# mkshing/e4t-diffusion

Hardware: NVIDIA H100
Metric: E4T pretrain images/sec @512^2 bs16 SD-v1.4 (higher is better)
Workload: dtype bf16

## Files before the change

e4t-diffusion_b200/csrc/attention_wgmma.cu:

```cuda
#include "attention.cuh"
#include "wgmma.cuh"

static constexpr int kWgThreads = 384;
static constexpr int kFwdStages = 3;
static constexpr int kTile128 = 128 * 128;
static constexpr int kTile64 = 64 * 128;
static constexpr size_t kMaxSmem = 227 * 1024;

__device__ __forceinline__ constexpr uint64_t kstep(int k, uint32_t panel) {
  return (uint64_t)((k / 4) * (panel >> 4) + 2 * (k % 4));
}

__device__ __forceinline__ uint8_t* align1024(uint8_t* p) {
  return p + ((1024u - (smem_u32(p) & 1023u)) & 1023u);
}

template <int DH>
struct FwdSmem {
  static constexpr int P = (DH + 63) / 64;
  static constexpr uint32_t kTile = P * kTile128;
  static constexpr uint32_t kStage = 2 * kTile;
  static constexpr uint32_t kOffBar = kTile + kFwdStages * kStage;
  static constexpr size_t bytes = 1024 + kOffBar + 8 * (1 + 2 * kFwdStages);
  static constexpr uint32_t kLboV = P > 1 ? kTile128 : kTile64;
  static_assert(bytes <= kMaxSmem, "forward shared memory");
};

template <int DH>
struct BwdSmem {
  static constexpr int P = (DH + 63) / 64, BQ = 64;
  static constexpr int kStages = P > 1 ? 2 : 3;
  static constexpr uint32_t kKV = P * kTile128;
  static constexpr uint32_t kQ = P * kTile64;
  static constexpr uint32_t kStage = 2 * kQ;
  static constexpr uint32_t kOffQ = 2 * kKV;
  static constexpr uint32_t kOffdS = kOffQ + kStages * kStage;
  static constexpr uint32_t kOffdQ = kOffdS + 2 * kTile128;
  static constexpr uint32_t kdQBytes = BQ * DH * 4;
  static constexpr uint32_t kOffL = kOffdQ + 2 * kdQBytes;
  static constexpr uint32_t kOffBar = kOffL + kStages * 2 * BQ * 4;
  static constexpr size_t bytes = 1024 + kOffBar + 8 * (1 + 2 * kStages + 4);
  static constexpr uint32_t kLboK = P > 1 ? kTile128 : kTile64;
  static_assert(kOffdQ % 128 == 0 && kdQBytes % 128 == 0 && kOffL % 16 == 0 && kOffBar % 8 == 0, "smem layout");
  static_assert(bytes <= kMaxSmem, "backward shared memory");
};

__device__ __forceinline__ void fwd_softmax(float (&s)[64], float (&m)[2], float (&l)[2], float (&alpha)[2], float sl2) {
#pragma unroll
  for (int hr = 0; hr < 2; ++hr) {
    float mx = -INFINITY;
#pragma unroll
    for (int j = 0; j < 16; ++j) mx = fmaxf(mx, fmaxf(s[4 * j + 2 * hr], s[4 * j + 2 * hr + 1]));
    mx = fmaxf(mx, __shfl_xor_sync(0xffffffffu, mx, 1));
    mx = fmaxf(mx, __shfl_xor_sync(0xffffffffu, mx, 2));
    const float mnew = fmaxf(m[hr], mx * sl2);
    alpha[hr] = ex2_approx(m[hr] - mnew);
    m[hr] = mnew;
    float rs = 0.f;
#pragma unroll
    for (int j = 0; j < 16; ++j)
#pragma unroll
      for (int e = 0; e < 2; ++e) {
        const float p = ex2_approx(fmaf(s[4 * j + 2 * hr + e], sl2, -mnew));
        s[4 * j + 2 * hr + e] = p;
        rs += p;
      }
    l[hr] = l[hr] * alpha[hr] + rs;
  }
}

template <int NJ>
__device__ __forceinline__ void pack_acc(const float* s, uint32_t* p) {
#pragma unroll
  for (int i = 0; i < 2 * NJ; ++i) p[i] = pack_bf16(s[2 * i], s[2 * i + 1]);
}

template <int DH>
__global__ void __launch_bounds__(kWgThreads, 1)
attn_wgmma_fwd_kernel(const __grid_constant__ CUtensorMap mapQ, const __grid_constant__ CUtensorMap mapK,
                      const __grid_constant__ CUtensorMap mapV, const AttnArgs a) {
  using L = FwdSmem<DH>;
  constexpr int KS = (DH + 15) / 16, NO = DH;
  constexpr uint32_t kStage = L::kStage;
  extern __shared__ __align__(1024) uint8_t smem_raw[];
  uint8_t* smem = align1024(smem_raw);
  uint64_t* q_bar = reinterpret_cast<uint64_t*>(smem + L::kOffBar);
  uint64_t* full_bar = q_bar + 1;
  uint64_t* empty_bar = full_bar + kFwdStages;
  const int wg = threadIdx.x >> 7;
  const int b = blockIdx.z, h = blockIdx.y, q0 = blockIdx.x * 128;
  const int nblk = a.M / 128;
  if (threadIdx.x == 0) {
    tma_prefetch_desc(&mapQ);
    tma_prefetch_desc(&mapK);
    tma_prefetch_desc(&mapV);
    mbar_init(q_bar, 1);
    for (int i = 0; i < kFwdStages; ++i) {
      mbar_init(&full_bar[i], 1);
      mbar_init(&empty_bar[i], 256);
    }
    fence_mbar_init();
  }
  __syncthreads();

  if (wg == 0) {
    setmaxnreg_dec<24>();
    if (threadIdx.x != 0) return;
    mbar_expect_tx(q_bar, L::kTile);
#pragma unroll
    for (int pn = 0; pn < L::P; ++pn) tma_load_4d(smem + pn * kTile128, &mapQ, q_bar, 64 * pn, h, q0, b);
    int s = 0;
    uint32_t ph = 0;
    for (int j = 0; j < nblk; ++j) {
      mbar_wait(&empty_bar[s], ph ^ 1u);
// ... 141 lines not shown
    }
    for (int i = 0; i < 2; ++i) {
      mbar_init(&ds_full[i], 256);
      mbar_init(&ds_empty[i], 128);
    }
    fence_mbar_init();
  }
  __syncthreads();
  const uint32_t s0 = smem_u32(smem);

  if (wg == 0) {
    setmaxnreg_dec<72>();
    auto load_block = [&](int i) {
      const int s = i % kBwdStages;
      mbar_wait(&empty_bar[s], ((uint32_t)(i / kBwdStages) & 1u) ^ 1u);
      uint8_t* sQ = smem + kOffQ + s * kStage;
      mbar_expect_tx(&full_bar[s], kStage + 2 * BQ * 4);
#pragma unroll
      for (int pn = 0; pn < L::P; ++pn) {
        tma_load_4d(sQ + pn * kTile64, &mapQ, &full_bar[s], 64 * pn, h, i * BQ, b);
        tma_load_4d(sQ + L::kQ + pn * kTile64, &mapdO, &full_bar[s], 64 * pn, h, i * BQ, b);
      }
      bulk_load_1d(sL + s * 2 * BQ, a.LSE + bh * a.N + i * BQ, BQ * 4, &full_bar[s]);
      bulk_load_1d(sL + s * 2 * BQ + BQ, a.Dv + bh * a.N + i * BQ, BQ * 4, &full_bar[s]);
    };
    if (threadIdx.x == 0) {
      mbar_expect_tx(kv_bar, 2 * L::kKV);
#pragma unroll
      for (int pn = 0; pn < L::P; ++pn) {
        tma_load_4d(smem + pn * kTile128, &mapK, kv_bar, 64 * pn, h, k0, b);
        tma_load_4d(smem + L::kKV + pn * kTile128, &mapV, kv_bar, 64 * pn, h, k0, b);
      }
      for (int i = 0; i < kBwdStages - 1 && i < nq; ++i) load_block(i);
    }
    __syncwarp();
    const uint64_t descS = wgmma_desc(s0 + kOffdS, kTile64, 1024);
    const uint64_t descK = wgmma_desc(s0, L::kLboK, 1024);
    mbar_wait(kv_bar, 0);
    float dq[NO / 2];
    for (int i = 0; i < nq; ++i) {
      const int buf = i & 1;
      if (threadIdx.x == 0 && i + kBwdStages - 1 < nq) load_block(i + kBwdStages - 1);
      __syncwarp();
      mbar_wait(&ds_full[buf], (uint32_t)(i >> 1) & 1u);
      const uint64_t da = descS + (uint64_t)(buf * (kTile128 >> 4));
      wgmma_fence();
#pragma unroll
      for (int kk = 0; kk < 8; ++kk)
        Wgmma<NO, 1, 1>::mma(dq, da + (uint64_t)(kk * (2048 >> 4)), descK + (uint64_t)(kk * (2048 >> 4)), kk > 0);
      wgmma_commit();
      wgmma_wait<0>();
      reg_fence<NO / 2>(dq);
      mbar_arrive(&ds_empty[buf]);
      if (threadIdx.x == 0) tma_store_wait_read<1>();
      named_bar_sync(1, 128);
      float* stg = reinterpret_cast<float*>(smem + kOffdQ + buf * kdQBytes);
#pragma unroll
      for (int hr = 0; hr < 2; ++hr) {
        float* row = stg + (16 * warp + (lane >> 2) + 8 * hr) * DH + 2 * (lane & 3);
#pragma unroll
        for (int dt = 0; dt < DH / 8; ++dt)
          *reinterpret_cast<float2*>(row + 8 * dt) =
              make_float2(dq[4 * dt + 2 * hr] * a.scale, dq[4 * dt + 2 * hr + 1] * a.scale);
      }
      fence_proxy_async_smem();
      named_bar_sync(1, 128);
      if (threadIdx.x == 0) {
        tma_reduce_add_3d(&mapdQ, stg, h * DH, i * BQ, b);
        tma_store_commit();
      }
    }
    if (threadIdx.x == 0) tma_store_wait_all();
    return;
  }

  setmaxnreg_inc<216>();
  const int cw = wg - 1;
  const uint64_t descKa = wgmma_desc(s0 + kTile64 * cw, 16, 1024);
  const uint64_t descVa = wgmma_desc(s0 + L::kKV + kTile64 * cw, 16, 1024);
  const uint64_t descQk = wgmma_desc(s0 + kOffQ, 16, 1024);
  const uint64_t descQm = wgmma_desc(s0 + kOffQ, kTile64, 1024);
  const float sl2 = a.scale * kLog2e;
  float st[32], dpt[32], dk[NO / 2], dv[NO / 2];
  uint32_t pp[16], ps[16];
#pragma unroll
  for (int i = 0; i < NO / 2; ++i) dk[i] = dv[i] = 0.f;
  const int r0 = 64 * cw + 16 * warp + (lane >> 2);
  mbar_wait(kv_bar, 0);
  for (int i = 0; i < nq; ++i) {
    const int s = i % kBwdStages, buf = i & 1;
    mbar_wait(&full_bar[s], (uint32_t)(i / kBwdStages) & 1u);
    const uint64_t so = (uint64_t)(s * (kStage >> 4));
    reg_fence<32>(st);
    reg_fence<32>(dpt);
    wgmma_fence();
#pragma unroll
    for (int k = 0; k < KS; ++k)
      Wgmma<64, 0, 0>::mma(st, descKa + kstep(k, kTile128), descQk + so + kstep(k, kTile64), k > 0);
    wgmma_commit();
#pragma unroll
    for (int k = 0; k < KS; ++k)
      Wgmma<64, 0, 0>::mma(dpt, descVa + kstep(k, kTile128), descQk + so + (L::kQ >> 4) + kstep(k, kTile64), k > 0);
    wgmma_commit();
    const float* l_s = sL + s * 2 * BQ + 2 * (lane & 3);
    wgmma_wait<1>();
    reg_fence<32>(st);
#pragma unroll
    for (int j = 0; j < 8; ++j) {
      const float2 l = *reinterpret_cast<const float2*>(l_s + 8 * j);
      const float l0 = l.x * kLog2e, l1 = l.y * kLog2e;
      st[4 * j] = ex2_approx(fmaf(st[4 * j], sl2, -l0));
      st[4 * j + 1] = ex2_approx(fmaf(st[4 * j + 1], sl2, -l1));
      st[4 * j + 2] = ex2_approx(fmaf(st[4 * j + 2], sl2, -l0));
      st[4 * j + 3] = ex2_approx(fmaf(st[4 * j + 3], sl2, -l1));
    }
    pack_acc<8>(st, pp);
    wgmma_wait<0>();
    reg_fence<32>(dpt);
#pragma unroll
    for (int j = 0; j < 8; ++j) {
      const float2 d = *reinterpret_cast<const float2*>(l_s + BQ + 8 * j);
      dpt[4 * j] = st[4 * j] * (dpt[4 * j] - d.x);
      dpt[4 * j + 1] = st[4 * j + 1] * (dpt[4 * j + 1] - d.y);
      dpt[4 * j + 2] = st[4 * j + 2] * (dpt[4 * j + 2] - d.x);
      dpt[4 * j + 3] = st[4 * j + 3] * (dpt[4 * j + 3] - d.y);
    }
    pack_acc<8>(dpt, ps);
    mbar_wait(&ds_empty[buf], ((uint32_t)(i >> 1) & 1u) ^ 1u);
    uint8_t* sdS = smem + kOffdS + buf * kTile128;
#pragma unroll
    for (int j = 0; j < 8; ++j) {
      *reinterpret_cast<uint32_t*>(sdS + sw128_off(r0, j) + 4 * (lane & 3)) = ps[2 * j];
      *reinterpret_cast<uint32_t*>(sdS + sw128_off(r0 + 8, j) + 4 * (lane & 3)) = ps[2 * j + 1];
    }
    fence_proxy_async_smem();
    mbar_arrive(&ds_full[buf]);
    reg_fence<NO / 2>(dk);
    reg_fence<NO / 2>(dv);
    wgmma_fence();
#pragma unroll
    for (int kq = 0; kq < 4; ++kq)
      WgmmaRS<NO, 1>::mma(dv, pp + 4 * kq, descQm + so + (uint64_t)((L::kQ >> 4) + kq * (2048 >> 4)), 1);
#pragma unroll
    for (int kq = 0; kq < 4; ++kq) WgmmaRS<NO, 1>::mma(dk, ps + 4 * kq, descQm + so + (uint64_t)(kq * (2048 >> 4)), 1);
    wgmma_commit();
    wgmma_wait<0>();
    reg_fence<NO / 2>(dk);
    reg_fence<NO / 2>(dv);
    reg_fence_u32<16>(pp);
    reg_fence_u32<16>(ps);
    mbar_arrive(&empty_bar[s]);
  }
#pragma unroll
  for (int hr = 0; hr < 2; ++hr) {
    const int key = k0 + r0 + 8 * hr;
    bf16* dkr = a.dK + b * a.dk_bs + (long long)key * a.lddk + h * DH + 2 * (lane & 3);
    bf16* dvr = a.dV + b * a.dv_bs + (long long)key * a.lddv + h * DH + 2 * (lane & 3);
#pragma unroll
    for (int dt = 0; dt < DH / 8; ++dt) {
      *reinterpret_cast<uint32_t*>(dkr + 8 * dt) = pack_bf16(dk[4 * dt + 2 * hr] * a.scale, dk[4 * dt + 2 * hr + 1] * a.scale);
      *reinterpret_cast<uint32_t*>(dvr + 8 * dt) = pack_bf16(dv[4 * dt + 2 * hr], dv[4 * dt + 2 * hr + 1]);
    }
  }
}

bool attn_wgmma_shape_ok(int B, int H, int N, int M, int dh) {
  if (!(dh == 40 || dh == 64 || dh == 80) || N < 512 || M < 512 || N % 128 != 0 || M % 128 != 0) return false;
  if (dh == 40) return true;
  int sms = 0, dev = 0;
  cudaGetDevice(&dev);
  cudaDeviceGetAttribute(&sms, cudaDevAttrMultiProcessorCount, dev);
  if (sms <= 0) sms = 132;
  return 2LL * (N / 128) * H * B >= sms;
}

static int head_map(CUtensorMap* m, const bf16* p, const AttnArgs& a, int tokens, long long ld, long long bs, int rows) {
  E4T_CHECK(((uintptr_t)p & 15) == 0 && ld % 8 == 0 && bs % 8 == 0,
            "attention (wgmma): tensors must be 16-byte aligned with strides that are multiples of 8 elements");
  const uint64_t dims[4] = {(uint64_t)a.dh, (uint64_t)a.H, (uint64_t)tokens, (uint64_t)a.B};
  const uint64_t str[3] = {(uint64_t)a.dh * 2, (uint64_t)ld * 2, (uint64_t)bs * 2};
  const uint32_t box[4] = {64, 1, (uint32_t)rows, 1};
  return e4t_tmap_encode(m, p, 4, dims, str, box, 2);
}

int attn_wgmma_fwd(const AttnArgs& a, cudaStream_t st) {
  CUtensorMap mQ, mK, mV;
  if (int e = head_map(&mQ, a.Q, a, a.N, a.ldq, a.q_bs, 128)) return e;
  if (int e = head_map(&mK, a.K, a, a.M, a.ldk, a.k_bs, 128)) return e;
  if (int e = head_map(&mV, a.V, a, a.M, a.ldv, a.v_bs, 128)) return e;
  E4T_CHECK(a.ldo % 2 == 0 && a.o_bs % 2 == 0, "attention (wgmma): output strides must be even");
  const size_t smem = a.dh == 40 ? FwdSmem<40>::bytes : a.dh == 64 ? FwdSmem<64>::bytes : FwdSmem<80>::bytes;
  auto kernel = a.dh == 40   ? attn_wgmma_fwd_kernel<40>
                : a.dh == 64 ? attn_wgmma_fwd_kernel<64>
                             : attn_wgmma_fwd_kernel<80>;
  E4T_CUDA(cudaFuncSetAttribute(kernel, cudaFuncAttributeMaxDynamicSharedMemorySize, (int)smem));
  kernel<<<dim3(a.N / 128, a.H, a.B), kWgThreads, smem, st>>>(mQ, mK, mV, a);
  E4T_COUNT_LAUNCH();
  E4T_LAUNCH_CHECK();
  return 0;
}

int attn_wgmma_bwd(const AttnArgs& a, cudaStream_t st) {
  CUtensorMap mQ, mK, mV, mdO, mdQ;
  if (int e = head_map(&mQ, a.Q, a, a.N, a.ldq, a.q_bs, 64)) return e;
  if (int e = head_map(&mK, a.K, a, a.M, a.ldk, a.k_bs, 128)) return e;
  if (int e = head_map(&mV, a.V, a, a.M, a.ldv, a.v_bs, 128)) return e;
  if (int e = head_map(&mdO, a.dO, a, a.N, a.lddo, a.do_bs, 64)) return e;
  {
    const uint64_t C = (uint64_t)a.H * a.dh;
    const uint64_t dims[3] = {C, (uint64_t)a.N, (uint64_t)a.B};
    const uint64_t str[2] = {C * 4, (uint64_t)a.N * C * 4};
    const uint32_t box[3] = {(uint32_t)a.dh, 64, 1};
    E4T_CHECK(((uintptr_t)a.dQacc & 15) == 0 && ((uintptr_t)a.LSE & 15) == 0 && ((uintptr_t)a.Dv & 15) == 0,
              "attention (wgmma): LSE, D and dQ scratch must be 16-byte aligned");
    if (int e = e4t_tmap_encode(&mdQ, a.dQacc, 3, dims, str, box, 4, 0)) return e;
  }
  E4T_CHECK(a.lddk % 2 == 0 && a.dk_bs % 2 == 0 && a.lddv % 2 == 0 && a.dv_bs % 2 == 0,
            "attention (wgmma): gradient strides must be even");
  const size_t smem = a.dh == 40 ? BwdSmem<40>::bytes : a.dh == 64 ? BwdSmem<64>::bytes : BwdSmem<80>::bytes;
  auto kernel = a.dh == 40   ? attn_wgmma_bwd_kernel<40>
                : a.dh == 64 ? attn_wgmma_bwd_kernel<64>
                             : attn_wgmma_bwd_kernel<80>;
  E4T_CUDA(cudaFuncSetAttribute(kernel, cudaFuncAttributeMaxDynamicSharedMemorySize, (int)smem));
  kernel<<<dim3(a.M / 128, a.H, a.B), kWgThreads, smem, st>>>(mQ, mK, mV, mdO, mdQ, a);
  E4T_COUNT_LAUNCH();
  E4T_LAUNCH_CHECK();
  return 0;
}
```

e4t-diffusion_b200/csrc/common.cuh:

```cuda
#pragma once
#include <cuda.h>
#include <cuda_runtime.h>
#include <cuda_bf16.h>
#include <stdint.h>
#include <stdio.h>
#include <string.h>

typedef __nv_bfloat16 bf16;

extern thread_local char g_e4t_err[512];
int e4t_set_error(const char* fmt, ...);

#define E4T_CHECK(cond, ...)                                   \
  do {                                                         \
    if (!(cond)) return e4t_set_error(__VA_ARGS__);            \
  } while (0)

#define E4T_CUDA(call)                                                                  \
  do {                                                                                  \
    cudaError_t _e = (call);                                                            \
    if (_e != cudaSuccess)                                                              \
      return e4t_set_error("%s:%d CUDA error %s: %s", __FILE__, __LINE__, #call,        \
                           cudaGetErrorString(_e));                                     \
  } while (0)
// ... 76 lines not shown
  asm volatile(
      "cp.async.bulk.tensor.2d.shared::cluster.global.mbarrier::complete_tx::bytes [%0], [%1, {%3, %4}], [%2];"
      ::"r"(smem_u32(smem)), "l"(reinterpret_cast<uint64_t>(m)), "r"(smem_u32(bar)), "r"(c0), "r"(c1)
      : "memory");
}
__device__ __forceinline__ void tma_load_3d(void* smem, const CUtensorMap* m, uint64_t* bar, int c0, int c1,
                                            int c2) {
  asm volatile(
      "cp.async.bulk.tensor.3d.shared::cluster.global.mbarrier::complete_tx::bytes [%0], [%1, {%3, %4, %5}], [%2];"
      ::"r"(smem_u32(smem)), "l"(reinterpret_cast<uint64_t>(m)), "r"(smem_u32(bar)), "r"(c0), "r"(c1), "r"(c2)
      : "memory");
}
__device__ __forceinline__ void tma_load_4d(void* smem, const CUtensorMap* m, uint64_t* bar, int c0, int c1,
                                            int c2, int c3) {
  asm volatile(
      "cp.async.bulk.tensor.4d.shared::cluster.global.mbarrier::complete_tx::bytes [%0], [%1, {%3, %4, %5, %6}], "
      "[%2];" ::"r"(smem_u32(smem)),
      "l"(reinterpret_cast<uint64_t>(m)), "r"(smem_u32(bar)), "r"(c0), "r"(c1), "r"(c2), "r"(c3)
      : "memory");
}
__device__ __forceinline__ void tma_load_im2col_4d(void* smem, const CUtensorMap* m, uint64_t* bar, int c, int w,
                                                   int h, int n, int off_w, int off_h) {
  asm volatile(
      "cp.async.bulk.tensor.4d.shared::cluster.global.im2col.mbarrier::complete_tx::bytes [%0], [%1, {%3, %4, %5, "
      "%6}], [%2], {%7, %8};" ::"r"(smem_u32(smem)),
      "l"(reinterpret_cast<uint64_t>(m)), "r"(smem_u32(bar)), "r"(c), "r"(w), "r"(h), "r"(n),
      "h"((uint16_t)off_w), "h"((uint16_t)off_h)
      : "memory");
}

__device__ __forceinline__ void bulk_load_1d(void* smem, const void* g, uint32_t bytes, uint64_t* bar) {
  asm volatile("cp.async.bulk.shared::cluster.global.mbarrier::complete_tx::bytes [%0], [%1], %2, [%3];" ::"r"(
                   smem_u32(smem)),
               "l"(g), "r"(bytes), "r"(smem_u32(bar))
               : "memory");
}

__device__ __forceinline__ void tma_store_3d(const CUtensorMap* m, const void* smem, int c0, int c1, int c2) {
  asm volatile("cp.async.bulk.tensor.3d.global.shared::cta.bulk_group [%0, {%2, %3, %4}], [%1];" ::"l"(
                   reinterpret_cast<uint64_t>(m)),
               "r"(smem_u32(smem)), "r"(c0), "r"(c1), "r"(c2)
               : "memory");
}
__device__ __forceinline__ void tma_reduce_add_3d(const CUtensorMap* m, const void* smem, int c0, int c1, int c2) {
  asm volatile("cp.reduce.async.bulk.tensor.3d.global.shared::cta.add.tile.bulk_group [%0, {%2, %3, %4}], [%1];" ::"l"(
                   reinterpret_cast<uint64_t>(m)),
               "r"(smem_u32(smem)), "r"(c0), "r"(c1), "r"(c2)
               : "memory");
}
__device__ __forceinline__ void tma_store_commit() { asm volatile("cp.async.bulk.commit_group;" ::: "memory"); }
template <int N>
__device__ __forceinline__ void tma_store_wait_read() {
  asm volatile("cp.async.bulk.wait_group.read %0;" ::"n"(N) : "memory");
}
__device__ __forceinline__ void tma_store_wait_all() { asm volatile("cp.async.bulk.wait_group 0;" ::: "memory"); }

__device__ __forceinline__ uint64_t wgmma_desc(uint32_t saddr, uint32_t lbo_bytes, uint32_t sbo_bytes) {
  uint64_t d = 0;
  d |= (uint64_t)((saddr & 0x3FFFFu) >> 4);
  d |= (uint64_t)((lbo_bytes >> 4) & 0x3FFFu) << 16;
  d |= (uint64_t)((sbo_bytes >> 4) & 0x3FFFu) << 32;
  d |= 1ull << 62;
  return d;
}
__device__ __forceinline__ void wgmma_fence() { asm volatile("wgmma.fence.sync.aligned;" ::: "memory"); }
__device__ __forceinline__ void wgmma_commit() { asm volatile("wgmma.commit_group.sync.aligned;" ::: "memory"); }
template <int N>
__device__ __forceinline__ void wgmma_wait() {
  asm volatile("wgmma.wait_group.sync.aligned %0;" ::"n"(N) : "memory");
}
template <int R>
__device__ __forceinline__ void reg_fence(float* d) {
#pragma unroll
  for (int i = 0; i < R; ++i) asm volatile("" : "+f"(d[i])::"memory");
}
template <int R>
__device__ __forceinline__ void reg_fence_u32(uint32_t* a) {
#pragma unroll
  for (int i = 0; i < R; ++i) asm volatile("" : "+r"(a[i])::"memory");
}
__device__ __forceinline__ void named_bar_sync(uint32_t id, uint32_t nthreads) {
  asm volatile("bar.sync %0, %1;" ::"r"(id), "r"(nthreads) : "memory");
}
template <int R>
__device__ __forceinline__ void setmaxnreg_dec() {
  asm volatile("setmaxnreg.dec.sync.aligned.u32 %0;" ::"n"(R));
}
template <int R>
__device__ __forceinline__ void setmaxnreg_inc() {
  asm volatile("setmaxnreg.inc.sync.aligned.u32 %0;" ::"n"(R));
}

__device__ __forceinline__ void ldsm_x4(uint32_t addr, uint32_t* r) {
  asm volatile("ldmatrix.sync.aligned.m8n8.x4.shared.b16 {%0, %1, %2, %3}, [%4];"
               : "=r"(r[0]), "=r"(r[1]), "=r"(r[2]), "=r"(r[3])
               : "r"(addr));
}
__device__ __forceinline__ void ldsm_x4_t(uint32_t addr, uint32_t* r) {
  asm volatile("ldmatrix.sync.aligned.m8n8.x4.trans.shared.b16 {%0, %1, %2, %3}, [%4];"
               : "=r"(r[0]), "=r"(r[1]), "=r"(r[2]), "=r"(r[3])
               : "r"(addr));
}
__device__ __forceinline__ void mma16816(float* d, const uint32_t* a, const uint32_t* b) {
  asm volatile(
      "mma.sync.aligned.m16n8k16.row.col.f32.bf16.bf16.f32 {%0, %1, %2, %3}, {%4, %5, %6, %7}, {%8, %9}, "
      "{%0, %1, %2, %3};"
      : "+f"(d[0]), "+f"(d[1]), "+f"(d[2]), "+f"(d[3])
      : "r"(a[0]), "r"(a[1]), "r"(a[2]), "r"(a[3]), "r"(b[0]), "r"(b[1]));
}
__device__ __forceinline__ void cp_async16(uint32_t dst, const void* src, uint32_t src_bytes) {
  asm volatile("cp.async.cg.shared.global [%0], [%1], 16, %2;" ::"r"(dst), "l"(src), "r"(src_bytes) : "memory");
}
__device__ __forceinline__ void cp_async_commit() { asm volatile("cp.async.commit_group;" ::: "memory"); }
template <int N>
__device__ __forceinline__ void cp_async_wait() {
  asm volatile("cp.async.wait_group %0;" ::"n"(N) : "memory");
}

__device__ __forceinline__ uint32_t sw128_off(uint32_t r, uint32_t c16) {
  return r * 128u + ((c16 ^ (r & 7u)) << 4);
}

__device__ __forceinline__ float warp_sum(float v) {
#pragma unroll
  for (int o = 16; o > 0; o >>= 1) v += __shfl_xor_sync(0xffffffffu, v, o);
  return v;
}
__device__ __forceinline__ float warp_max(float v) {
#pragma unroll
  for (int o = 16; o > 0; o >>= 1) v = fmaxf(v, __shfl_xor_sync(0xffffffffu, v, o));
  return v;
}
__device__ __forceinline__ uint32_t pack_bf16(float a, float b) {
  __nv_bfloat162 t = __floats2bfloat162_rn(a, b);
  return *reinterpret_cast<uint32_t*>(&t);
}
__device__ __forceinline__ float2 unpack_bf16(uint32_t u) {
  __nv_bfloat162 t = *reinterpret_cast<__nv_bfloat162*>(&u);
  return __bfloat1622float2(t);
}
__device__ __forceinline__ float ex2_approx(float x) {
  float y;
  asm("ex2.approx.ftz.f32 %0, %1;" : "=f"(y) : "f"(x));
  return y;
}
__device__ __forceinline__ float silu_f(float x) { return x / (1.f + __expf(-x)); }
#endif
```

e4t-diffusion_b200/csrc/norm.cu:

```cuda
#include "common.cuh"
#include <stdlib.h>

static constexpr int kGNMaxThreads = 320;

struct GNChan {
  float mean, rstd, gamma, beta;
};

__device__ __forceinline__ float sigmoid_fast(float y) { return __fdividef(1.f, 1.f + __expf(-y)); }
__device__ __forceinline__ float silu_fast(float y) { return y * sigmoid_fast(y); }
__device__ __forceinline__ float silu_grad(float y) {
  const float sg = sigmoid_fast(y);
  return sg * (1.f + y * (1.f - sg));
}
__device__ __forceinline__ void unpack8(const uint4& u, float* f) {
  const float2 a = unpack_bf16(u.x), b = unpack_bf16(u.y), c = unpack_bf16(u.z), d = unpack_bf16(u.w);
  f[0] = a.x; f[1] = a.y; f[2] = b.x; f[3] = b.y; f[4] = c.x; f[5] = c.y; f[6] = d.x; f[7] = d.y;
}
__device__ __forceinline__ uint4 pack8(const float* f) {
  return make_uint4(pack_bf16(f[0], f[1]), pack_bf16(f[2], f[3]), pack_bf16(f[4], f[5]), pack_bf16(f[6], f[7]));
}
__device__ __forceinline__ void gn_thread_chan(GNChan* ch, const float* __restrict__ stats,
                                               const float* __restrict__ gamma, const float* __restrict__ beta, int b,
                                               int c0, int C, int G, float inv_n, float eps) {
  const int cpg = C / G;
#pragma unroll
  for (int j = 0; j < 8; ++j) {
    const int g = (c0 + j) / cpg;
    const float2 mr = gn_mean_rstd(stats + ((long)b * G + g) * kGNStat, inv_n, eps);
    ch[j].mean = mr.x;
    ch[j].rstd = mr.y;
    ch[j].gamma = gamma[c0 + j];
    ch[j].beta = beta[c0 + j];
  }
}

template <int MODE>
__global__ void __launch_bounds__(kGNMaxThreads)
gn_stats_kernel(const bf16* __restrict__ x, const bf16* __restrict__ dy, const float* __restrict__ fstats,
                const float* __restrict__ gamma, const float* __restrict__ beta, float* __restrict__ sums, int HW,
                int C, int G, int rows_per_cta, float eps, int act) {
  extern __shared__ __align__(16) uint8_t gsm[];
  float2* schan = reinterpret_cast<float2*>(gsm);
  const int b = blockIdx.y;
  const int vpr = C / 8;
  const int cv = threadIdx.x % vpr, rl = threadIdx.x / vpr, rstep = blockDim.x / vpr;
  const int c0 = cv * 8;
  const int r0 = blockIdx.x * rows_per_cta;
  const int r1 = min(HW, r0 + rows_per_cta);
  const int cpg = C / G;
  const bf16* ximg = x + ((long)b * HW) * C;
  GNChan ch[8];
  float piv[8];
  if (MODE == 1) gn_thread_chan(ch, fstats, gamma, beta, b, c0, C, G, 1.f / ((float)HW * (float)cpg), eps);
#pragma unroll
  for (int j = 0; j < 8; ++j) piv[j] = MODE == 0 ? __bfloat162float(ximg[(c0 + j) / cpg * cpg]) : 0.f;
  __syncthreads();
  float a0[8], a1[8];
#pragma unroll
  for (int j = 0; j < 8; ++j) a0[j] = a1[j] = 0.f;
  const bf16* xb = ximg + c0;
  const bf16* db = MODE == 1 ? dy + ((long)b * HW) * C + c0 : nullptr;
#pragma unroll 4
  for (int r = r0 + rl; r < r1; r += rstep) {
    float xv[8];
    unpack8(__ldg(reinterpret_cast<const uint4*>(xb + (long)r * C)), xv);
    if (MODE == 0) {
#pragma unroll
      for (int j = 0; j < 8; ++j) {
        const float d = xv[j] - piv[j];
        a0[j] += d;
        a1[j] += d * d;
      }
    } else {
      float dv[8];
      unpack8(__ldg(reinterpret_cast<const uint4*>(db + (long)r * C)), dv);
#pragma unroll
      for (int j = 0; j < 8; ++j) {
        const float xh = (xv[j] - ch[j].mean) * ch[j].rstd;
        float g = dv[j] * ch[j].gamma;
        if (act) g *= silu_grad(xh * ch[j].gamma + ch[j].beta);
        a0[j] += g;
        a1[j] += g * xh;
// ... 24 lines not shown
gn_apply_kernel(const bf16* __restrict__ x, const bf16* __restrict__ dy, const float* __restrict__ fstats,
                const float* __restrict__ bstats, const float* __restrict__ gamma, const float* __restrict__ beta,
                bf16* __restrict__ out, int HW, int C, int G, int rows_per_cta, float eps, int act) {
  const int b = blockIdx.y;
  const float inv_n = 1.f / ((float)HW * (float)(C / G));
  const int vpr = C / 8;
  const int cv = threadIdx.x % vpr, rl = threadIdx.x / vpr, rstep = blockDim.x / vpr;
  const int c0 = cv * 8;
  GNChan ch[8];
  gn_thread_chan(ch, fstats, gamma, beta, b, c0, C, G, inv_n, eps);
  float scale[8], shift[8], m1[8], m2[8];
  const int cpg = C / G;
#pragma unroll
  for (int j = 0; j < 8; ++j) {
    scale[j] = ch[j].rstd * ch[j].gamma;
    shift[j] = ch[j].beta - ch[j].mean * scale[j];
    if (MODE == 1) {
      const int g = (c0 + j) / cpg;
      m1[j] = bstats[((long)b * G + g) * 2] * inv_n;
      m2[j] = bstats[((long)b * G + g) * 2 + 1] * inv_n;
    }
  }
  const int r0 = blockIdx.x * rows_per_cta;
  const int r1 = min(HW, r0 + rows_per_cta);
  const long base = ((long)b * HW) * C + c0;
#pragma unroll 4
  for (int r = r0 + rl; r < r1; r += rstep) {
    float xv[8], o[8];
    unpack8(*reinterpret_cast<const uint4*>(x + base + (long)r * C), xv);
    if (MODE == 0) {
#pragma unroll
      for (int j = 0; j < 8; ++j) {
        o[j] = fmaf(xv[j], scale[j], shift[j]);
        if (act) o[j] = silu_fast(o[j]);
      }
    } else {
      float dv[8];
      unpack8(*reinterpret_cast<const uint4*>(dy + base + (long)r * C), dv);
#pragma unroll
      for (int j = 0; j < 8; ++j) {
        const float xh = (xv[j] - ch[j].mean) * ch[j].rstd;
        float g = dv[j] * ch[j].gamma;
        if (act) g *= silu_grad(fmaf(xv[j], scale[j], shift[j]));
        o[j] = ch[j].rstd * (g - m1[j] - xh * m2[j]);
      }
    }
    *reinterpret_cast<uint4*>(out + base + (long)r * C) = pack8(o);
  }
}

static int gn_env(const char* name) {
  const char* e = getenv(name);
  return e ? atoi(e) : 0;
}
template <typename K>
static int gn_rows_per_cta(K kernel, int threads, size_t smem_per_rl, int C, int B, int HW) {
  const int forced = gn_env("E4T_GN_ROWS");
  if (forced > 0) return forced;
  int occ = 0;
  const size_t smem = smem_per_rl * (size_t)(threads / (C / 8));
  if (cudaOccupancyMaxActiveBlocksPerMultiprocessor(&occ, kernel, threads, smem) != cudaSuccess || occ < 1) occ = 4;
  int sms = 0, dev = 0;
  cudaGetDevice(&dev);
  cudaDeviceGetAttribute(&sms, cudaDevAttrMultiProcessorCount, dev);
  if (sms <= 0) sms = 132;
  const long target = (long)sms * occ;
  long chunks = target / B;
  if (chunks < 1) chunks = 1;
  if (chunks > HW) chunks = HW;
  int rows = cdiv(HW, chunks);
  const int rstep = threads / (C / 8);
  if (rows < rstep) rows = rstep;
  return rows;
}
static int gn_block(int C) {
  const int vpr = C / 8;
  int target = gn_env("E4T_GN_THREADS");
  if (target <= 0 || target > kGNMaxThreads) target = 256;
  int k = target / vpr;
  if (k < 1) k = 1;
  return vpr * k;
}

extern "C" int e4t_groupnorm_fwd(const void* x, const float* gamma, const float* beta, void* y, float* stats, int B,
                                 int HW, int C, int G, float eps, int act_silu, void* stream_) {
  cudaStream_t st = (cudaStream_t)stream_;
  E4T_CHECK(C % G == 0 && C % 8 == 0 && C / 8 <= kGNMaxThreads, "e4t_groupnorm_fwd: unsupported C=%d G=%d", C, G);
  E4T_CUDA(cudaMemsetAsync(stats, 0, (size_t)B * G * kGNStat * sizeof(float), st));
  const int threads = gn_block(C);
  const int rows = gn_rows_per_cta(gn_stats_kernel<0>, threads, (size_t)C * sizeof(float2), C, B, HW);
  dim3 grid(cdiv(HW, rows), B);
  gn_stats_kernel<0><<<grid, threads, (size_t)(threads / (C / 8)) * C * sizeof(float2), st>>>((const bf16*)x, nullptr, nullptr, nullptr,
                                                                        nullptr, stats, HW, C, G, rows, eps, 0);
  E4T_COUNT_LAUNCH();
  E4T_LAUNCH_CHECK();
  const int rows_a = gn_rows_per_cta(gn_apply_kernel<0>, threads, 0, C, B, HW);
  gn_apply_kernel<0><<<dim3(cdiv(HW, rows_a), B), threads, 0, st>>>((const bf16*)x, nullptr, stats, nullptr, gamma, beta,
                                                                    (bf16*)y, HW, C, G, rows_a, eps, act_silu);
  E4T_COUNT_LAUNCH();
  E4T_LAUNCH_CHECK();
  return 0;
}

extern "C" int e4t_groupnorm_bwd(const void* x, const void* dy, const float* gamma, const float* beta,
                                 const float* stats, void* dx, float* scratch, int B, int HW, int C, int G, float eps,
                                 int act_silu, void* stream_) {
  cudaStream_t st = (cudaStream_t)stream_;
  E4T_CHECK(C % G == 0 && C % 8 == 0 && C / 8 <= kGNMaxThreads, "e4t_groupnorm_bwd: unsupported C=%d G=%d", C, G);
  E4T_CUDA(cudaMemsetAsync(scratch, 0, (size_t)B * G * 2 * sizeof(float), st));
  const int threads = gn_block(C);
  const int rows = gn_rows_per_cta(gn_stats_kernel<1>, threads, (size_t)C * sizeof(float2), C, B, HW);
  dim3 grid(cdiv(HW, rows), B);
  gn_stats_kernel<1><<<grid, threads, (size_t)(threads / (C / 8)) * C * sizeof(float2), st>>>((const bf16*)x, (const bf16*)dy, stats, gamma,
                                                                        beta, scratch, HW, C, G, rows, eps, act_silu);
  E4T_COUNT_LAUNCH();
  E4T_LAUNCH_CHECK();
  const int rows_a = gn_rows_per_cta(gn_apply_kernel<1>, threads, 0, C, B, HW);
  gn_apply_kernel<1><<<dim3(cdiv(HW, rows_a), B), threads, 0, st>>>((const bf16*)x, (const bf16*)dy, stats, scratch, gamma,
                                                                    beta, (bf16*)dx, HW, C, G, rows_a, eps, act_silu);
  E4T_COUNT_LAUNCH();
  E4T_LAUNCH_CHECK();
  return 0;
}

template <int MODE, int kLNMaxIter>
__global__ void __launch_bounds__(256)
ln_kernel(const bf16* __restrict__ x, const bf16* __restrict__ dy, const float* __restrict__ gamma,
          const float* __restrict__ beta, bf16* __restrict__ out, float* __restrict__ stats, long rows, int C,
          float eps) {
  const long row = (long)blockIdx.x * (blockDim.x >> 5) + (threadIdx.x >> 5);
  if (row >= rows) return;
  const int lane = threadIdx.x & 31;
  const int nv = C / 8;
  float v[kLNMaxIter][8];
  const bf16* xr = x + row * C;
#pragma unroll
  for (int it = 0; it < kLNMaxIter; ++it) {
    const int vi = lane + it * 32;
    if (vi < nv) {
      const uint4 u = *reinterpret_cast<const uint4*>(xr + vi * 8);
      const float2 a = unpack_bf16(u.x), b = unpack_bf16(u.y), c = unpack_bf16(u.z), d = unpack_bf16(u.w);
      v[it][0] = a.x; v[it][1] = a.y; v[it][2] = b.x; v[it][3] = b.y;
      v[it][4] = c.x; v[it][5] = c.y; v[it][6] = d.x; v[it][7] = d.y;
    } else {
#pragma unroll
      for (int j = 0; j < 8; ++j) v[it][j] = 0.f;
    }
  }
  float mean, rstd;
  if (MODE == 0) {
    float s = 0.f;
#pragma unroll
    for (int it = 0; it < kLNMaxIter; ++it)
#pragma unroll
      for (int j = 0; j < 8; ++j) s += v[it][j];
    mean = warp_sum(s) / (float)C;
    float q = 0.f;
#pragma unroll
    for (int it = 0; it < kLNMaxIter; ++it) {
      const int vi = lane + it * 32;
      if (vi < nv) {
#pragma unroll
        for (int j = 0; j < 8; ++j) {
          const float d = v[it][j] - mean;
          q += d * d;
        }
      }
    }
    rstd = rsqrtf(warp_sum(q) / (float)C + eps);
    if (lane == 0) {
      stats[row * 2] = mean;
      stats[row * 2 + 1] = rstd;
    }
  } else {
    mean = stats[row * 2];
    rstd = stats[row * 2 + 1];
  }
  if (MODE == 0) {
#pragma unroll
    for (int it = 0; it < kLNMaxIter; ++it) {
      const int vi = lane + it * 32;
      if (vi < nv) {
        const float4 g0 = *reinterpret_cast<const float4*>(gamma + vi * 8);
        const float4 g1 = *reinterpret_cast<const float4*>(gamma + vi * 8 + 4);
        const float4 b0 = *reinterpret_cast<const float4*>(beta + vi * 8);
        const float4 b1 = *reinterpret_cast<const float4*>(beta + vi * 8 + 4);
        const float gg[8] = {g0.x, g0.y, g0.z, g0.w, g1.x, g1.y, g1.z, g1.w};
        const float bb[8] = {b0.x, b0.y, b0.z, b0.w, b1.x, b1.y, b1.z, b1.w};
        float o[8];
#pragma unroll
        for (int j = 0; j < 8; ++j) o[j] = (v[it][j] - mean) * rstd * gg[j] + bb[j];
// ... 73 lines not shown
```

Measured before the change: 113.5.

## Software-pipeline attention backward for head dim 40 with ping-pong warpgroup scheduling

For head dim 40, the backward consumer loop now issues the S/dP GEMMs for the next Q tile before the dV/dK GEMMs of the previous tile. This overlaps the softmax-exp and dS work with tensor-core MMAs. The two consumer warpgroups also take turns issuing WGMMAs via named barriers, in ping-pong fashion, and the pipeline deepens to 4 stages. The cost is double-buffered pp/ps registers, more shared memory, and extra barrier synchronization. There is a risk of register pressure or barrier deadlock if nq is small.

Result: faster. 114.7, median of 6 (+1.0%).

```diff
diff --git a/e4t-diffusion_b200/csrc/attention_wgmma.cu b/e4t-diffusion_b200/csrc/attention_wgmma.cu
--- a/e4t-diffusion_b200/csrc/attention_wgmma.cu
+++ b/e4t-diffusion_b200/csrc/attention_wgmma.cu
@@ -1,3 +1,5 @@
+#include <type_traits>
+
 #include "attention.cuh"
 #include "wgmma.cuh"
 
@@ -29,7 +31,8 @@
 template <int DH>
 struct BwdSmem {
   static constexpr int P = (DH + 63) / 64, BQ = 64;
-  static constexpr int kStages = P > 1 ? 2 : 3;
+  static constexpr bool kPipelined = DH == 40;
+  static constexpr int kStages = kPipelined ? 4 : P > 1 ? 2 : 3;
   static constexpr uint32_t kKV = P * kTile128;
   static constexpr uint32_t kQ = P * kTile64;
   static constexpr uint32_t kStage = 2 * kQ;
@@ -337,14 +340,11 @@
   const uint64_t descQm = wgmma_desc(s0 + kOffQ, kTile64, 1024);
   const float sl2 = a.scale * kLog2e;
   float st[32], dpt[32], dk[NO / 2], dv[NO / 2];
-  uint32_t pp[16], ps[16];
 #pragma unroll
   for (int i = 0; i < NO / 2; ++i) dk[i] = dv[i] = 0.f;
   const int r0 = 64 * cw + 16 * warp + (lane >> 2);
-  mbar_wait(kv_bar, 0);
-  for (int i = 0; i < nq; ++i) {
-    const int s = i % kBwdStages, buf = i & 1;
-    mbar_wait(&full_bar[s], (uint32_t)(i / kBwdStages) & 1u);
+
+  auto issue_s_dp = [&](int s) {
     const uint64_t so = (uint64_t)(s * (kStage >> 4));
     reg_fence<32>(st);
     reg_fence<32>(dpt);
@@ -357,8 +357,9 @@
     for (int k = 0; k < KS; ++k)
       Wgmma<64, 0, 0>::mma(dpt, descVa + kstep(k, kTile128), descQk + so + (L::kQ >> 4) + kstep(k, kTile64), k > 0);
     wgmma_commit();
+  };
+  auto exp_p = [&](int s, uint32_t (&pp)[16]) {
     const float* l_s = sL + s * 2 * BQ + 2 * (lane & 3);
-    wgmma_wait<1>();
     reg_fence<32>(st);
 #pragma unroll
     for (int j = 0; j < 8; ++j) {
@@ -370,7 +371,10 @@
       st[4 * j + 3] = ex2_approx(fmaf(st[4 * j + 3], sl2, -l1));
     }
     pack_acc<8>(st, pp);
-    wgmma_wait<0>();
+  };
+  auto ds_store = [&](int i, int s, uint32_t (&ps)[16]) {
+    const float* l_s = sL + s * 2 * BQ + 2 * (lane & 3);
+    const int buf = i & 1;
     reg_fence<32>(dpt);
 #pragma unroll
     for (int j = 0; j < 8; ++j) {
@@ -390,6 +394,9 @@
     }
     fence_proxy_async_smem();
     mbar_arrive(&ds_full[buf]);
+  };
+  auto issue_dv_dk = [&](int s, uint32_t (&pp)[16], uint32_t (&ps)[16]) {
+    const uint64_t so = (uint64_t)(s * (kStage >> 4));
     reg_fence<NO / 2>(dk);
     reg_fence<NO / 2>(dv);
     wgmma_fence();
@@ -399,12 +406,67 @@
 #pragma unroll
     for (int kq = 0; kq < 4; ++kq) WgmmaRS<NO, 1>::mma(dk, ps + 4 * kq, descQm + so + (uint64_t)(kq * (2048 >> 4)), 1);
     wgmma_commit();
+  };
+  auto full_wait = [&](int i) { mbar_wait(&full_bar[i % kBwdStages], (uint32_t)(i / kBwdStages) & 1u); };
+
+  mbar_wait(kv_bar, 0);
+  if constexpr (!L::kPipelined) {
+    uint32_t pp[16], ps[16];
+    for (int i = 0; i < nq; ++i) {
+      const int s = i % kBwdStages;
+      full_wait(i);
+      issue_s_dp(s);
+      wgmma_wait<1>();
+      exp_p(s, pp);
+      wgmma_wait<0>();
+      ds_store(i, s, ps);
+      issue_dv_dk(s, pp, ps);
+      wgmma_wait<0>();
+      reg_fence<NO / 2>(dk);
+      reg_fence<NO / 2>(dv);
+      reg_fence_u32<16>(pp);
+      reg_fence_u32<16>(ps);
+      mbar_arrive(&empty_bar[s]);
+    }
+  } else {
+    auto turn_wait = [&]() { named_bar_sync(2 + cw, 256); };
+    auto turn_pass = [&]() { named_bar_arrive(3 - cw, 256); };
+    uint32_t pp0[16], ps0[16], pp1[16], ps1[16];
+    auto block = [&](auto first, int i, uint32_t (&pp)[16], uint32_t (&ps)[16], uint32_t (&pp_prev)[16],
+                     uint32_t (&ps_prev)[16]) {
+      constexpr bool kFirst = decltype(first)::value;
+      const int s = i % kBwdStages;
+      full_wait(i);
+      turn_wait();
+      issue_s_dp(s);
+      if constexpr (!kFirst) issue_dv_dk((i - 1) % kBwdStages, pp_prev, ps_prev);
+      if (cw == 0 || i + 1 < nq) turn_pass();
+      wgmma_wait<kFirst ? 1 : 2>();
+      exp_p(s, pp);
+      wgmma_wait<kFirst ? 0 : 1>();
+      ds_store(i, s, ps);
+      if constexpr (!kFirst) {
+        wgmma_wait<0>();
+        reg_fence<NO / 2>(dk);
+        reg_fence<NO / 2>(dv);
+        reg_fence_u32<16>(pp_prev);
+        reg_fence_u32<16>(ps_prev);
+        mbar_arrive(&empty_bar[(i - 1) % kBwdStages]);
+      }
+    };
+    if (cw == 1) turn_pass();
+    block(std::true_type(), 0, pp0, ps0, pp1, ps1);
+    for (int i = 1; i + 1 < nq; i += 2) {
+      block(std::false_type(), i, pp1, ps1, pp0, ps0);
+      block(std::false_type(), i + 1, pp0, ps0, pp1, ps1);
+    }
+    block(std::false_type(), nq - 1, pp1, ps1, pp0, ps0);
+    issue_dv_dk((nq - 1) % kBwdStages, pp1, ps1);
     wgmma_wait<0>();
     reg_fence<NO / 2>(dk);
     reg_fence<NO / 2>(dv);
-    reg_fence_u32<16>(pp);
-    reg_fence_u32<16>(ps);
-    mbar_arrive(&empty_bar[s]);
+    reg_fence_u32<16>(pp1);
+    reg_fence_u32<16>(ps1);
   }
 #pragma unroll
   for (int hr = 0; hr < 2; ++hr) {
diff --git a/e4t-diffusion_b200/csrc/common.cuh b/e4t-diffusion_b200/csrc/common.cuh
--- a/e4t-diffusion_b200/csrc/common.cuh
+++ b/e4t-diffusion_b200/csrc/common.cuh
@@ -182,6 +182,9 @@
 __device__ __forceinline__ void named_bar_sync(uint32_t id, uint32_t nthreads) {
   asm volatile("bar.sync %0, %1;" ::"r"(id), "r"(nthreads) : "memory");
 }
+__device__ __forceinline__ void named_bar_arrive(uint32_t id, uint32_t nthreads) {
+  asm volatile("bar.arrive %0, %1;" ::"r"(id), "r"(nthreads) : "memory");
+}
 template <int R>
 __device__ __forceinline__ void setmaxnreg_dec() {
   asm volatile("setmaxnreg.dec.sync.aligned.u32 %0;" ::"n"(R));
```

## Fuse GroupNorm stats and apply into one thread-block-cluster kernel with DSMEM reduction

Applied to the files above, without the earlier changes.

Replaces the memset + stats kernel + apply kernel sequence for GroupNorm forward and backward with a single kernel launched as 16-CTA clusters per image. Each CTA caches its rows in shared memory, reduces per-group partial sums, and combines them across the cluster through distributed shared memory before normalizing. This removes two launches, the global atomic stats pass, and the second read of x/dy for cached rows. The cost is large shared-memory use per CTA, a fixed cluster size of 16 (non-portable), and a grid of only B*16 CTAs, which may limit occupancy at large HW.

New measurement: 112.8 before, 111.9 after, median of 6. No clear change (-0.8%).

```diff
diff --git a/e4t-diffusion_b200/csrc/norm.cu b/e4t-diffusion_b200/csrc/norm.cu
--- a/e4t-diffusion_b200/csrc/norm.cu
+++ b/e4t-diffusion_b200/csrc/norm.cu
@@ -1,4 +1,5 @@
 #include "common.cuh"
+#include <cooperative_groups.h>
 #include <stdlib.h>
 
 static constexpr int kGNMaxThreads = 320;
@@ -189,10 +190,237 @@
   return vpr * k;
 }
 
+
+static constexpr int kGNClusterThreads = 256;
+static constexpr int kGNCluster = 16;
+static constexpr size_t kGNClusterSmem = 113 * 1024;
+
+template <int MODE>
+struct GNCol {
+  float piv[8];
+  float mean[8], rstd[8], gamma[8], beta[8];
+  float a0[8], a1[8];
+
+  __device__ __forceinline__ void accumulate(const uint4& ux, const uint4& ud, int act) {
+    float xv[8];
+    unpack8(ux, xv);
+    if (MODE == 0) {
+#pragma unroll
+      for (int j = 0; j < 8; ++j) {
+        const float d = xv[j] - piv[j];
+        a0[j] += d;
+        a1[j] += d * d;
+      }
+    } else {
+      float dv[8];
+      unpack8(ud, dv);
+#pragma unroll
+      for (int j = 0; j < 8; ++j) {
+        const float xh = (xv[j] - mean[j]) * rstd[j];
+        float g = dv[j] * gamma[j];
+        if (act) g *= silu_grad(xh * gamma[j] + beta[j]);
+        a0[j] += g;
+        a1[j] += g * xh;
+      }
+    }
+  }
+};
+
+template <int MODE>
+__global__ void __launch_bounds__(kGNClusterThreads, 2)
+gn_cluster_kernel(const bf16* __restrict__ x, const bf16* __restrict__ dy, const float* __restrict__ gamma,
+                  const float* __restrict__ beta, float* __restrict__ stats, bf16* __restrict__ out, int HW, int C,
+                  int G, int rows_per, int cap, float eps, int act) {
+  namespace cg = cooperative_groups;
+  cg::cluster_group cluster = cg::this_cluster();
+  extern __shared__ __align__(16) uint8_t gsm[];
+  const int vpr = C / 8;
+  const int cv = threadIdx.x % vpr, rl = threadIdx.x / vpr, rstep = blockDim.x / vpr;
+  const int c0 = cv * 8;
+  const int cpg = C / G;
+  float2* part = reinterpret_cast<float2*>(gsm);
+  float2* tot = part + G;
+  float2* schan = tot + G;
+  uint4* sx = reinterpret_cast<uint4*>(schan + rstep * C);
+  uint4* sd = sx + (size_t)cap * vpr;
+  const int b = blockIdx.y;
+  const float inv_n = 1.f / ((float)HW * (float)cpg);
+  const int r0 = min(HW, (int)cluster.block_rank() * rows_per);
+  const int r1 = min(HW, r0 + rows_per);
+  const int rm = min(r1, r0 + cap);
+  const long img = (long)b * HW * C;
+  const uint4* xg = reinterpret_cast<const uint4*>(x + img + c0);
+  const uint4* dg = MODE == 1 ? reinterpret_cast<const uint4*>(dy + img + c0) : nullptr;
+  const int vstride = vpr;
+
+  GNCol<MODE> t;
+#pragma unroll
+  for (int j = 0; j < 8; ++j) {
+    t.a0[j] = t.a1[j] = 0.f;
+    t.gamma[j] = gamma[c0 + j];
+    t.beta[j] = beta[c0 + j];
+    if (MODE == 0) {
+      t.piv[j] = __bfloat162float(x[img + (c0 + j) / cpg * cpg]);
+    } else {
+      const float2 mr = gn_mean_rstd(stats + ((long)b * G + (c0 + j) / cpg) * kGNStat, inv_n, eps);
+      t.mean[j] = mr.x;
+      t.rstd[j] = mr.y;
+    }
+  }
+  const uint4 zero = make_uint4(0, 0, 0, 0);
+#pragma unroll 4
+  for (int r = r0 + rl; r < rm; r += rstep) {
+    const uint4 ux = __ldg(xg + (long)r * vstride);
+    const uint4 ud = MODE == 1 ? __ldg(dg + (long)r * vstride) : zero;
+    sx[(r - r0) * vpr + cv] = ux;
+    if (MODE == 1) sd[(r - r0) * vpr + cv] = ud;
+    t.accumulate(ux, ud, act);
+  }
+#pragma unroll 4
+  for (int r = rm + rl; r < r1; r += rstep)
+    t.accumulate(__ldg(xg + (long)r * vstride), MODE == 1 ? __ldg(dg + (long)r * vstride) : zero, act);
+
+#pragma unroll
+  for (int j = 0; j < 8; ++j) schan[rl * C + c0 + j] = make_float2(t.a0[j], t.a1[j]);
+  __syncthreads();
+  for (int g = threadIdx.x; g < G; g += blockDim.x) {
+    float s = 0.f, ss = 0.f;
+    for (int q = 0; q < rstep; ++q)
+      for (int i = 0; i < cpg; ++i) {
+        const float2 p = schan[q * C + g * cpg + i];
+        s += p.x;
+        ss += p.y;
+      }
+    part[g] = make_float2(s, ss);
+  }
+  cluster.sync();
+  const int kc = (int)cluster.num_blocks();
+  for (int g = threadIdx.x; g < G; g += blockDim.x) {
+    float s = 0.f, ss = 0.f;
+    for (int q = 0; q < kc; ++q) {
+      const float2 p = cluster.map_shared_rank(part, q)[g];
+      s += p.x;
+      ss += p.y;
+    }
+    tot[g] = make_float2(s, ss);
+    if (MODE == 0 && cluster.block_rank() == 0) {
+      float* sg = stats + ((long)b * G + g) * kGNStat;
+      sg[0] = __bfloat162float(x[img + g * cpg]);
+      sg[1] = s;
+      sg[2] = ss;
+    }
+  }
+  cluster.barrier_arrive();
+  __syncthreads();
+
+  float scale[8], shift[8], m1[8], m2[8];
+#pragma unroll
+  for (int j = 0; j < 8; ++j) {
+    const float2 tg = tot[(c0 + j) / cpg];
+    if (MODE == 0) {
+      const float st[kGNStat] = {t.piv[j], tg.x, tg.y};
+      const float2 mr = gn_mean_rstd(st, inv_n, eps);
+      t.mean[j] = mr.x;
+      t.rstd[j] = mr.y;
+    } else {
+      m1[j] = tg.x * inv_n;
+      m2[j] = tg.y * inv_n;
+    }
+    scale[j] = t.rstd[j] * t.gamma[j];
+    shift[j] = t.beta[j] - t.mean[j] * scale[j];
+  }
+  uint4* og = reinterpret_cast<uint4*>(out + img + c0);
+  auto emit = [&](int r, const uint4& ux, const uint4& ud) {
+    float xv[8], o[8];
+    unpack8(ux, xv);
+    if (MODE == 0) {
+#pragma unroll
+      for (int j = 0; j < 8; ++j) {
+        o[j] = fmaf(xv[j], scale[j], shift[j]);
+        if (act) o[j] = silu_fast(o[j]);
+      }
+    } else {
+      float dv[8];
+      unpack8(ud, dv);
+#pragma unroll
+      for (int j = 0; j < 8; ++j) {
+        const float xh = (xv[j] - t.mean[j]) * t.rstd[j];
+        float g = dv[j] * t.gamma[j];
+        if (act) g *= silu_grad(fmaf(xv[j], scale[j], shift[j]));
+        o[j] = t.rstd[j] * (g - m1[j] - xh * m2[j]);
+      }
+    }
+    og[(long)r * vstride] = pack8(o);
+  };
+#pragma unroll 4
+  for (int r = rm + rl; r < r1; r += rstep)
+    emit(r, __ldg(xg + (long)r * vstride), MODE == 1 ? __ldg(dg + (long)r * vstride) : zero);
+#pragma unroll 4
+  for (int r = r0 + rl; r < rm; r += rstep)
+    emit(r, sx[(r - r0) * vpr + cv], MODE == 1 ? sd[(r - r0) * vpr + cv] : zero);
+  cluster.barrier_wait();
+}
+
+struct GNPlan {
+  int threads, rows_per, cap;
+  size_t smem;
+};
+static GNPlan gn_plan(int MODE, int HW, int C, int G) {
+  GNPlan p;
+  const int vpr = C / 8;
+  p.threads = vpr * (kGNClusterThreads / vpr);
+  p.rows_per = cdiv(HW, kGNCluster);
+  const size_t fixed = 2 * (size_t)G * sizeof(float2) + (size_t)(p.threads / vpr) * C * sizeof(float2);
+  const size_t row_bytes = (size_t)C * sizeof(bf16) * (MODE == 0 ? 1 : 2);
+  const size_t room = fixed < kGNClusterSmem ? (kGNClusterSmem - fixed) / row_bytes : 0;
+  p.cap = (int)(room < (size_t)p.rows_per ? room : (size_t)p.rows_per);
+  p.smem = fixed + (size_t)p.cap * row_bytes;
+  return p;
+}
+
+template <int MODE>
+static int gn_launch(const void* x, const void* dy, const float* gamma, const float* beta, float* stats, void* out,
+                     int B, int HW, int C, int G, float eps, int act, cudaStream_t st) {
+  const GNPlan p = gn_plan(MODE, HW, C, G);
+  E4T_CHECK(p.smem <= kGNClusterSmem, "groupnorm: C=%d G=%d needs %zu bytes of shared memory", C, G, p.smem);
+  auto kernel = gn_cluster_kernel<MODE>;
+  static bool attr_set = false;
+  if (!attr_set) {
+    E4T_CUDA(cudaFuncSetAttribute(kernel, cudaFuncAttributeNonPortableClusterSizeAllowed, 1));
+    E4T_CUDA(cudaFuncSetAttribute(kernel, cudaFuncAttributeMaxDynamicSharedMemorySize, (int)kGNClusterSmem));
+    attr_set = true;
+  }
+  cudaLaunchConfig_t cfg = {};
+  cfg.gridDim = dim3(kGNCluster, B);
+  cfg.blockDim = dim3(p.threads);
+  cfg.dynamicSmemBytes = p.smem;
+  cfg.stream = st;
+  cudaLaunchAttribute attr[1];
+  attr[0].id = cudaLaunchAttributeClusterDimension;
+  attr[0].val.clusterDim.x = kGNCluster;
+  attr[0].val.clusterDim.y = 1;
+  attr[0].val.clusterDim.z = 1;
+  cfg.attrs = attr;
+  cfg.numAttrs = 1;
+  E4T_CUDA(cudaLaunchKernelEx(&cfg, kernel, (const bf16*)x, (const bf16*)dy, gamma, beta, stats, (bf16*)out, HW, C, G,
+                              p.rows_per, p.cap, eps, act));
+  E4T_COUNT_LAUNCH();
+  return 0;
+}
+
+static bool gn_use_cluster(int B, int C) {
+  int sms = 0, dev = 0;
+  cudaGetDevice(&dev);
+  cudaDeviceGetAttribute(&sms, cudaDevAttrMultiProcessorCount, dev);
+  if (sms <= 0) sms = 132;
+  return C / 8 <= kGNClusterThreads && (long)B * kGNCluster >= sms;
+}
+
 extern "C" int e4t_groupnorm_fwd(const void* x, const float* gamma, const float* beta, void* y, float* stats, int B,
                                  int HW, int C, int G, float eps, int act_silu, void* stream_) {
   cudaStream_t st = (cudaStream_t)stream_;
   E4T_CHECK(C % G == 0 && C % 8 == 0 && C / 8 <= kGNMaxThreads, "e4t_groupnorm_fwd: unsupported C=%d G=%d", C, G);
+  if (gn_use_cluster(B, C)) return gn_launch<0>(x, nullptr, gamma, beta, stats, y, B, HW, C, G, eps, act_silu, st);
   E4T_CUDA(cudaMemsetAsync(stats, 0, (size_t)B * G * kGNStat * sizeof(float), st));
   const int threads = gn_block(C);
   const int rows = gn_rows_per_cta(gn_stats_kernel<0>, threads, (size_t)C * sizeof(float2), C, B, HW);
@@ -214,6 +442,8 @@
                                  int act_silu, void* stream_) {
   cudaStream_t st = (cudaStream_t)stream_;
   E4T_CHECK(C % G == 0 && C % 8 == 0 && C / 8 <= kGNMaxThreads, "e4t_groupnorm_bwd: unsupported C=%d G=%d", C, G);
+  if (gn_use_cluster(B, C))
+    return gn_launch<1>(x, dy, gamma, beta, const_cast<float*>(stats), dx, B, HW, C, G, eps, act_silu, st);
   E4T_CUDA(cudaMemsetAsync(scratch, 0, (size_t)B * G * 2 * sizeof(float), st));
   const int threads = gn_block(C);
   const int rows = gn_rows_per_cta(gn_stats_kernel<1>, threads, (size_t)C * sizeof(float2), C, B, HW);
```
